# weiyithu/PV-RAFT

Hardware: NVIDIA H100
Metric: raft_sample_iters_per_sec (higher is better)
Workload: dtype f32

## Files before the change

### pvraft_b200/csrc/common.cuh

```cuda
#pragma once
#include <cstdlib>
#include <cuda_runtime.h>
#include <stdint.h>
#include <stdio.h>

#include "../../include/pvraft_b200.h"

namespace pvraft {

constexpr int kWarp = 32;
constexpr unsigned kFull = 0xffffffffu;
constexpr int kSmemBudget = 227 * 1024;

void set_error(const char* fmt, ...);
int fail(int code, const char* fmt, ...);
int check_launch(const char* what);
int sm_count();

template <typename Kernel>
inline int opt_in_smem(Kernel k, size_t bytes) {
    if (bytes > (size_t)kSmemBudget) return fail(PVRAFT_ERR_SMEM, "kernel needs %zu B of shared memory (> %d)", bytes, kSmemBudget);
    cudaError_t e = cudaFuncSetAttribute(k, cudaFuncAttributeMaxDynamicSharedMemorySize, (int)bytes);
    if (e != cudaSuccess) return fail((int)e, "cudaFuncSetAttribute(smem=%zu): %s", bytes, cudaGetErrorString(e));
    return 0;
}

__device__ __forceinline__ int lane_id() { return threadIdx.x & 31; }
__device__ __forceinline__ int warp_id() { return threadIdx.x >> 5; }

__device__ __forceinline__ float warp_max(float v) {
#pragma unroll
    for (int o = 16; o > 0; o >>= 1) v = fmaxf(v, __shfl_xor_sync(kFull, v, o));
    return v;
}
__device__ __forceinline__ float warp_min(float v) {
#pragma unroll
    for (int o = 16; o > 0; o >>= 1) v = fminf(v, __shfl_xor_sync(kFull, v, o));
    return v;
}
__device__ __forceinline__ double warp_sum(double v) {
#pragma unroll
    for (int o = 16; o > 0; o >>= 1) v += __shfl_xor_sync(kFull, v, o);
    return v;
}
__device__ __forceinline__ float warp_sum(float v) {
#pragma unroll
    for (int o = 16; o > 0; o >>= 1) v += __shfl_xor_sync(kFull, v, o);
    return v;
}

__device__ __forceinline__ float4 ld_stream_f4(const float4* p) {
    float4 r;
    asm volatile("ld.global.nc.L1::no_allocate.v4.f32 {%0,%1,%2,%3}, [%4];" : "=f"(r.x), "=f"(r.y), "=f"(r.z), "=f"(r.w) : "l"(p));
    return r;
}
__device__ __forceinline__ int4 ld_stream_i4(const int4* p) {
    int4 r;
    asm volatile("ld.global.nc.L1::no_allocate.v4.s32 {%0,%1,%2,%3}, [%4];" : "=r"(r.x), "=r"(r.y), "=r"(r.z), "=r"(r.w) : "l"(p));
    return r;
}

struct GnAffine {
    float scale, shift;
};
__device__ __forceinline__ GnAffine gn_affine(const double* stats_bg , double count,
                                              float gamma, float beta) {
    const double mean = stats_bg[0] / count;
    double var = stats_bg[1] / count - mean * mean;
    var = var < 0.0 ? 0.0 : var;
    const double rstd = rsqrt(var + 1e-5);
    GnAffine a;
    a.scale = (float)(rstd * (double)gamma);
    a.shift = (float)((double)beta - mean * rstd * (double)gamma);
    return a;
}

__device__ __forceinline__ void kahan_add(float& s, float& err, float y) {
    const float v = y - err, t = s + v;
    err = (t - s) - v;
    s = t;
}
__device__ __forceinline__ double kahan_value(float s, float err) { return (double)s - (double)err; }
__device__ __forceinline__ double pivot_sumsq(double sum_y, float p, float sdd, int n) {
    const double dp = p;
    return fma(dp, 2.0 * sum_y - (double)n * dp, (double)sdd);
}

__device__ __forceinline__ float apply_act(float x, int act, float slope) {
    if (act == PVRAFT_ACT_RELU) return fmaxf(x, 0.f);
    if (act == PVRAFT_ACT_LRELU) return x >= 0.f ? x : slope * x;
    return x;
}

struct ActCoef {
    float lo, slope;
};
__device__ __forceinline__ ActCoef act_coef(int act, float slope) {
    ActCoef c;
    c.lo = act == PVRAFT_ACT_NONE ? -INFINITY : 0.f;
    c.slope = act == PVRAFT_ACT_LRELU ? slope : 0.f;
    return c;
}
__device__ __forceinline__ float apply_act(float x, const ActCoef& c) { return fmaf(c.slope, fminf(x, 0.f), fmaxf(x, c.lo)); }

__device__ __forceinline__ float4 tc_gn_act4(float4 x, const float4& sc, const float4& sh, const ActCoef& act) {
    x.x = apply_act(fmaf(x.x, sc.x, sh.x), act);
    x.y = apply_act(fmaf(x.y, sc.y, sh.y), act);
    x.z = apply_act(fmaf(x.z, sc.z, sh.z), act);
    x.w = apply_act(fmaf(x.w, sc.w, sh.w), act);
    return x;
}

__device__ __forceinline__ float tsigmoid(float x) { return 1.f / (1.f + expf(-x)); }
__device__ __forceinline__ float tgru_blend(float z, float h, float q_pre) { return (1.f - z) * h + z * tanhf(q_pre); }

__host__ __device__ __forceinline__ void split_range(long long total, int parts, int w, long long& begin, long long& end) {
    const long long per = (total + parts - 1) / parts;
    begin = per * w;
    end = begin + per;
    if (begin > total) begin = total;
    if (end > total) end = total;
}

__device__ __forceinline__ void pdl_trigger() { asm volatile("griddepcontrol.launch_dependents;" ::: "memory"); }
__device__ __forceinline__ void pdl_wait() { asm volatile("griddepcontrol.wait;" ::: "memory"); }
template <typename... KArgs, typename... Args>
inline cudaError_t launch_pdl(void (*kernel)(KArgs...), int grid, int block, size_t smem, cudaStream_t stream, Args... args) {
    cudaLaunchConfig_t cfg{};
    cfg.gridDim = dim3((unsigned)grid);
    cfg.blockDim = dim3((unsigned)block);
    cfg.dynamicSmemBytes = smem;
    cfg.stream = stream;
    cudaLaunchAttribute attr[1];
    attr[0].id = cudaLaunchAttributeProgrammaticStreamSerialization;
    attr[0].val.programmaticStreamSerializationAllowed = 1;
    cfg.attrs = attr;
    cfg.numAttrs = 1;
    return cudaLaunchKernelEx(&cfg, kernel, KArgs(args)...);
}

}
```

### pvraft_b200/csrc/update_chain.cu

```cuda
#include "tma.cuh"
#include "wgmma.cuh"

namespace pvraft {

constexpr int kChThreads = 288;
constexpr int kChProducerWarp = 8;
constexpr int kChWBytes = 128 * kTcKB * 4;
template <bool BF16> struct ChRing {
    static constexpr int stages = BF16 ? 4 : 2;
    static constexpr int w_off = BF16 ? kTcABytes + 2 * kTcABf16Bytes : 2 * kTcABytes;
    static constexpr int stage_bytes = BF16 ? w_off + kChWBytes / 2 : w_off + 2 * kChWBytes;
};
constexpr int kChBufBytes = 2 * kTcABytes;
constexpr int kChSteps = 24;
enum ChSrc { CH_Y1 = 0, CH_KFEAT, CH_CFLOW, CH_NET, CH_INP, CH_X, CH_Y };

struct ChainParams {
    const double* y1_stats;
    const float *gn_gamma, *gn_beta;
    double gn_count;
    float gn_slope;
    const float *flow, *net;
    const float *b_cc, *b_m, *b_z, *b_r, *b_q;
    float *net_out, *p_out;
    int M, pts_per_sample;
};
struct ChainMaps {
    CUtensorMap a[5];
    CUtensorMap w_hi[5], w_lo[5];
};

__device__ __forceinline__ int ch_layer(int i) { return i < 6 ? 0 : i < 10 ? 1 : i < 16 ? 2 : i < 22 ? 3 : 4; }
__device__ __forceinline__ int ch_src(int i) {
    constexpr unsigned long long pairs = (unsigned long long)CH_X | (unsigned long long)CH_CFLOW << 4 | (unsigned long long)CH_NET << 8 |
                                         (unsigned long long)CH_INP << 12 | (unsigned long long)CH_Y << 16 | (unsigned long long)CH_X << 20 |
                                         (unsigned long long)CH_INP << 24 | (unsigned long long)CH_Y << 28 | (unsigned long long)CH_X << 32;
    return i < 4 ? CH_Y1 : i < 6 ? CH_KFEAT : (int)((pairs >> (4 * ((i - 6) >> 1))) & 15u);
}
__device__ __forceinline__ int ch_skb(int i) {
    return i < 4 ? i : (i < 6 ? i - 4 : (i - 6) & 1);
}
__device__ __forceinline__ int ch_first(int layer) { return layer == 0 ? 0 : layer == 1 ? 6 : layer == 2 ? 10 : layer == 3 ? 16 : 22; }
__device__ __forceinline__ int ch_w_bytes(int layer, bool bf16) { return (layer == 2 ? 128 : 64) * kTcKB * (bf16 ? 2 : 4); }

__device__ __forceinline__ void ch_buf_store2(unsigned char* buf, int r, int c, float v0, float v1) {
    const int lc = (c & 31) >> 2;
    *reinterpret_cast<float2*>(buf + (c >> 5) * kTcABytes + r * 128 + ((lc ^ (r & 7)) << 4) + (c & 3) * 4) = make_float2(v0, v1);
}

template <int N, bool BF16>
__device__ __forceinline__ void ch_kblock(float (&acc)[64], int kb, int src, int skb, unsigned char* tiles, unsigned char* buf_x,
                                          unsigned char* buf_y, const float* g_scale, const float* g_shift, const ActCoef& iact,
                                          unsigned long long* s_full, unsigned long long* s_empty, TcCursor& cp, int grp, int t,
                                          int lane) {
    const int s = cp.s;
    mbar_wait(&s_full[s], cp.phase);
    unsigned char* st = tiles + (size_t)s * ChRing<BF16>::stage_bytes;
    const unsigned char* from = src == CH_X ? buf_x + skb * kTcABytes : src == CH_Y ? buf_y + skb * kTcABytes : st;
#pragma unroll
    for (int i = 0; i < 4; ++i) {
        const int c = t + i * 128, r = grp * 64 + (c >> 3), lc = c & 7;
        const int off = r * 128 + ((lc ^ (r & 7)) << 4);
        float4 x = *reinterpret_cast<const float4*>(from + off);
        if (src == CH_Y1) {
            const int k = skb * kTcKB + lc * 4;
            x = tc_gn_act4(x, *reinterpret_cast<const float4*>(g_scale + k), *reinterpret_cast<const float4*>(g_shift + k), iact);
        }
        if constexpr (BF16) tc_bf16_store(st + kTcABytes + grp * kTcABf16Bytes, c >> 3, lc, x);
        else tc_split_store(st, off, x);
    }
    asm volatile("fence.proxy.async.shared::cta;" ::: "memory");
    asm volatile("bar.sync %0, 128;" ::"r"(1 + grp) : "memory");
    const unsigned char* wb = st + ChRing<BF16>::w_off;
    wgmma_fence_regs(acc);
    wgmma_fence();
    if constexpr (BF16) tc_mma_kblock_bf16<N>(acc, wgmma_desc_bf16(st + kTcABytes + grp * kTcABf16Bytes), wgmma_desc_bf16(wb), kb);
    else tc_mma_kblock<N>(acc, wgmma_desc(st + grp * 64 * 128), wgmma_desc(st + kTcABytes + grp * 64 * 128), wgmma_desc(wb),
                          wgmma_desc(wb + N * kTcKB * 4), kb);
    wgmma_commit();
    wgmma_wait<0>();
    if (lane == 0) mbar_arrive(&s_empty[s]);
    cp.next(kChSteps, ChRing<BF16>::stages);
}
template <int N, bool BF16>
__device__ __forceinline__ void ch_layer_mma(float (&acc)[64], int i0, int nkb, unsigned char* tiles, unsigned char* buf_x,
                                             unsigned char* buf_y, const float* g_scale, const float* g_shift, const ActCoef& iact,
                                             unsigned long long* s_full, unsigned long long* s_empty, TcCursor& cp, int grp, int t,
                                             int lane) {
    for (int kb = 0; kb < nkb; ++kb)
        ch_kblock<N, BF16>(acc, kb, ch_src(i0 + kb), ch_skb(i0 + kb), tiles, buf_x, buf_y, g_scale, g_shift, iact, s_full, s_empty, cp, grp, t, lane);
    wgmma_fence_regs(acc);
}

template <bool BF16>
__global__ void __launch_bounds__(kChThreads, 1)
k_update_chain(const __grid_constant__ ChainMaps maps, const ChainParams p) {
    constexpr int kChStages = ChRing<BF16>::stages, kChStageBytes = ChRing<BF16>::stage_bytes;
    extern __shared__ __align__(1024) unsigned char smem_raw[];
    unsigned char* tiles = SMEM_ALIGN_1024(smem_raw);
    unsigned char* buf_x = tiles + (size_t)kChStages * kChStageBytes;
    unsigned char* buf_y = buf_x + kChBufBytes;
    float* s_scale = reinterpret_cast<float*>(buf_y + kChBufBytes);
    float* s_bias = s_scale + 2 * 256;
    __shared__ __align__(8) unsigned long long s_full[kChStages], s_empty[kChStages];
    const int warp = warp_id(), lane = lane_id();
    const int n_tiles = p.M / kTcM;
    const int my_tiles = blockIdx.x < n_tiles ? (n_tiles - 1 - blockIdx.x) / gridDim.x + 1 : 0;
    if (warp == kChProducerWarp && lane == 0) {
        for (int i = 0; i < 5; ++i) {
            prefetch_tensormap(&maps.a[i]);
            prefetch_tensormap(&maps.w_hi[i]);
            if constexpr (!BF16) prefetch_tensormap(&maps.w_lo[i]);
        }
        for (int s = 0; s < kChStages; ++s) { mbar_init(&s_full[s], 1); mbar_init(&s_empty[s], 8); }
        fence_mbarrier_init();
    }
    asm volatile("griddepcontrol.launch_dependents;" ::: "memory");
    __syncthreads();
    asm volatile("griddepcontrol.wait;" ::: "memory");
    if (threadIdx.x < 64) {
        const int c = threadIdx.x;
        s_bias[c] = __ldg(p.b_cc + c);
        s_bias[64 + c] = c < 61 ? __ldg(p.b_m + c) : 0.f;
        s_bias[128 + c] = __ldg(p.b_z + c);
        s_bias[192 + c] = __ldg(p.b_r + c);
        s_bias[256 + c] = __ldg(p.b_q + c);
    }
    __syncthreads();

    if (warp == kChProducerWarp) {
        if (lane == 0) {
            TcCursor cw;
            for (int step = 0; step < my_tiles * kChSteps; ++step, cw.next(kChSteps, kChStages)) {
                const int i = cw.kb, layer = ch_layer(i), src = ch_src(i);
                const int row0 = (blockIdx.x + cw.ti * gridDim.x) * kTcM;
                const int wb = ch_w_bytes(layer, BF16);
                const int lkb = i - ch_first(layer), skb = ch_skb(i);
                mbar_wait(&s_empty[cw.s], cw.phase ^ 1u);
                unsigned char* st = tiles + (size_t)cw.s * kChStageBytes;
                mbar_expect_tx(&s_full[cw.s], (unsigned)((src < CH_X ? kTcABytes : 0) + (BF16 ? 1 : 2) * wb));
                if (src < CH_X) tma_load_2d(st, &maps.a[src], &s_full[cw.s], skb * kTcKB, row0);
                tma_load_2d(st + ChRing<BF16>::w_off, &maps.w_hi[layer], &s_full[cw.s], lkb * kTcKB, 0);
                if constexpr (!BF16) tma_load_2d(st + ChRing<BF16>::w_off + wb, &maps.w_lo[layer], &s_full[cw.s], lkb * kTcKB, 0);
            }
        }
        return;
    }

    const int grp = warp >> 2, t = threadIdx.x & 127;
    float* g_scale = s_scale + grp * 256;
    float* g_shift = g_scale + 128;
    const ActCoef iact = act_coef(PVRAFT_ACT_LRELU, p.gn_slope);
    const ActCoef relu = act_coef(PVRAFT_ACT_RELU, 0.f), none = act_coef(PVRAFT_ACT_NONE, 0.f);
    const int tiles_per_sample = p.pts_per_sample / kTcM;
    const int rq = (warp & 3) * 16 + (lane >> 2);
    const int cq = 2 * (lane & 3);
    int table_sample = -1;
    TcCursor cp;
    float acc[64], z[32];
    for (int ti = 0; ti < my_tiles; ++ti) {
        const int tile = blockIdx.x + ti * gridDim.x;
        const int row0 = tile * kTcM;
        const int sample = tile / tiles_per_sample;
        if (sample != table_sample) {
            table_sample = sample;
            asm volatile("bar.sync %0, 128;" ::"r"(1 + grp) : "memory");
            const double* sp = p.y1_stats + (size_t)sample * 16 + (t / 16) * 2;
            const double st[2] = {__ldcg(sp), __ldcg(sp + 1)};
            const GnAffine af = gn_affine(st, p.gn_count, __ldg(p.gn_gamma + t), __ldg(p.gn_beta + t));
            g_scale[t] = af.scale;
            g_shift[t] = af.shift;
            asm volatile("bar.sync %0, 128;" ::"r"(1 + grp) : "memory");
        }
        const int r_lo = grp * 64 + rq;
        ch_layer_mma<64, BF16>(acc, 0, 6, tiles, buf_x, buf_y, g_scale, g_shift, iact, s_full, s_empty, cp, grp, t, lane);
#pragma unroll
        for (int j = 0; j < 8; ++j)
#pragma unroll
            for (int h = 0; h < 2; ++h) {
                const int c = 8 * j + cq;
                ch_buf_store2(buf_x, r_lo + 8 * h, c, apply_act(acc[4 * j + 2 * h] + s_bias[c], relu), apply_act(acc[4 * j + 2 * h + 1] + s_bias[c + 1], relu));
            }
        asm volatile("bar.sync %0, 128;" ::"r"(1 + grp) : "memory");
        ch_layer_mma<64, BF16>(acc, 6, 4, tiles, buf_x, buf_y, g_scale, g_shift, iact, s_full, s_empty, cp, grp, t, lane);
#pragma unroll
        for (int j = 0; j < 8; ++j)
#pragma unroll
            for (int h = 0; h < 2; ++h) {
                const int c = 8 * j + cq, r = r_lo + 8 * h;
                float v0 = apply_act(acc[4 * j + 2 * h] + s_bias[64 + c], relu), v1 = apply_act(acc[4 * j + 2 * h + 1] + s_bias[64 + c + 1], relu);
                if (c >= 60) {
                    const float* fl = p.flow + (size_t)(row0 + r) * 3;
                    if (c == 62) { v0 = __ldcg(fl + 1); v1 = __ldcg(fl + 2); } else { v1 = __ldcg(fl); }
                }
                ch_buf_store2(buf_y, r, c, v0, v1);
            }
        asm volatile("bar.sync %0, 128;" ::"r"(1 + grp) : "memory");
        ch_layer_mma<128, BF16>(acc, 10, 6, tiles, buf_x, buf_y, g_scale, g_shift, iact, s_full, s_empty, cp, grp, t, lane);
#pragma unroll
        for (int j = 0; j < 8; ++j)
#pragma unroll
            for (int h = 0; h < 2; ++h) {
                const int c = 8 * j + cq, r = r_lo + 8 * h;
                const float2 hv = __ldcg(reinterpret_cast<const float2*>(p.net + (size_t)(row0 + r) * 64 + c));
                z[4 * j + 2 * h] = tsigmoid(acc[4 * j + 2 * h] + s_bias[128 + c]);
                z[4 * j + 2 * h + 1] = tsigmoid(acc[4 * j + 2 * h + 1] + s_bias[128 + c + 1]);
                ch_buf_store2(buf_x, r, c, tsigmoid(acc[32 + 4 * j + 2 * h] + s_bias[192 + c]) * hv.x,
                              tsigmoid(acc[32 + 4 * j + 2 * h + 1] + s_bias[192 + c + 1]) * hv.y);
            }
        asm volatile("bar.sync %0, 128;" ::"r"(1 + grp) : "memory");
        ch_layer_mma<64, BF16>(acc, 16, 6, tiles, buf_x, buf_y, g_scale, g_shift, iact, s_full, s_empty, cp, grp, t, lane);
#pragma unroll
        for (int j = 0; j < 8; ++j)
#pragma unroll
            for (int h = 0; h < 2; ++h) {
                const int c = 8 * j + cq, r = r_lo + 8 * h;
                const size_t g = (size_t)(row0 + r) * 64 + c;
                const float2 hv = __ldcg(reinterpret_cast<const float2*>(p.net + g));
                const float o0 = tgru_blend(z[4 * j + 2 * h], hv.x, acc[4 * j + 2 * h] + s_bias[256 + c]);
                const float o1 = tgru_blend(z[4 * j + 2 * h + 1], hv.y, acc[4 * j + 2 * h + 1] + s_bias[256 + c + 1]);
                *reinterpret_cast<float2*>(p.net_out + g) = make_float2(o0, o1);
                ch_buf_store2(buf_x, r, c, o0, o1);
            }
        asm volatile("bar.sync %0, 128;" ::"r"(1 + grp) : "memory");
        ch_layer_mma<64, BF16>(acc, 22, 2, tiles, buf_x, buf_y, g_scale, g_shift, iact, s_full, s_empty, cp, grp, t, lane);
#pragma unroll
        for (int j = 0; j < 8; ++j)
#pragma unroll
            for (int h = 0; h < 2; ++h) {
                const int c = 8 * j + cq, r = r_lo + 8 * h;
                *reinterpret_cast<float2*>(p.p_out + (size_t)(row0 + r) * 64 + c) =
                    make_float2(apply_act(acc[4 * j + 2 * h] + 0.f, none), apply_act(acc[4 * j + 2 * h + 1] + 0.f, none));
            }
    }
}

}

using namespace pvraft;

extern "C" int pvraft_update_chain_fwd(const pvraft_update_chain_args* a, void* stream) {
    if (!a || !a->y1 || !a->y1_stats || !a->gn_gamma || !a->gn_beta || !a->kfeat || !a->cflow || !a->flow || !a->net || !a->inp ||
        !a->b_cc || !a->b_m || !a->b_z || !a->b_r || !a->b_q || !a->net_out || !a->p_out)
        return fail(PVRAFT_ERR_BAD_ARG, "update_chain: null pointer");
    const bool bf16 = a->w_bf16[0] != nullptr;
    for (int l = 0; l < 5; ++l) {
        if (bf16 ? (!a->w_bf16[l] || a->w_hi[l] || a->w_lo[l]) : (!a->w_hi[l] || !a->w_lo[l] || a->w_bf16[l]))
            return fail(PVRAFT_ERR_BAD_ARG, "update_chain: layer %d needs w_hi and w_lo (3xTF32) or w_bf16 (bf16), as every other layer", l);
    }
    if (a->B <= 0 || a->N <= 0) return fail(PVRAFT_ERR_BAD_ARG, "update_chain: bad shape (B=%d, N=%d)", a->B, a->N);
    if (a->N % kTcM) return fail(PVRAFT_ERR_UNSUPPORTED, "update_chain: points per sample (%d) must be a multiple of 128", a->N);
    if (a->hidden != 64 || a->context != 64 || a->y1_channels != 128)
        return fail(PVRAFT_ERR_UNSUPPORTED, "update_chain: built for hidden = context = 64 and 128 lookup features (got %d, %d, %d)",
                    a->hidden, a->context, a->y1_channels);
    if (a->net_out == a->net) return fail(PVRAFT_ERR_BAD_ARG, "update_chain: net_out must not alias net");
    const long long M = (long long)a->B * a->N;
    ChainMaps maps;
    const float* src[5] = {a->y1, a->kfeat, a->cflow, a->net, a->inp};
    const int width[5] = {128, 64, 64, 64, 64};
    const int n_pad[5] = {64, 64, 128, 64, 64}, k[5] = {192, 128, 192, 192, 64};
    int rc;
    for (int i = 0; i < 5; ++i) {
        if ((rc = make_tensor_map(&maps.a[i], src[i], M, width[i], width[i], kTcM, "update_chain"))) return rc;
        if (bf16) {
            if ((rc = make_tensor_map_bf16(&maps.w_hi[i], a->w_bf16[i], n_pad[i], k[i], k[i], n_pad[i], "update_chain"))) return rc;
            maps.w_lo[i] = maps.w_hi[i];
        } else if ((rc = make_tensor_map(&maps.w_hi[i], a->w_hi[i], n_pad[i], k[i], k[i], n_pad[i], "update_chain")) ||
                   (rc = make_tensor_map(&maps.w_lo[i], a->w_lo[i], n_pad[i], k[i], k[i], n_pad[i], "update_chain"))) {
            return rc;
        }
    }
    ChainParams p{};
    p.y1_stats = a->y1_stats; p.gn_gamma = a->gn_gamma; p.gn_beta = a->gn_beta; p.gn_count = a->gn_count; p.gn_slope = a->gn_slope;
    p.flow = a->flow; p.net = a->net;
    p.b_cc = a->b_cc; p.b_m = a->b_m; p.b_z = a->b_z; p.b_r = a->b_r; p.b_q = a->b_q;
    p.net_out = a->net_out; p.p_out = a->p_out;
    p.M = (int)M; p.pts_per_sample = a->N;
    const size_t ring = bf16 ? (size_t)ChRing<true>::stages * ChRing<true>::stage_bytes : (size_t)ChRing<false>::stages * ChRing<false>::stage_bytes;
    const size_t smem = ring + 2 * kChBufBytes + (2 * 256 + 5 * 64) * sizeof(float) + 1024;
    const auto kernel = bf16 ? k_update_chain<true> : k_update_chain<false>;
    if ((rc = opt_in_smem(kernel, smem))) return rc;
    const long long n_tiles = M / kTcM;
    const int grid = (int)(n_tiles < sm_count() ? n_tiles : sm_count());
    const cudaError_t le = launch_pdl(kernel, grid, kChThreads, smem, (cudaStream_t)stream, maps, p);
    if (le != cudaSuccess) return fail((int)le, "update_chain: launch failed: %s", cudaGetErrorString(le));
    return check_launch("update_chain");
}
```

Baseline: 9922.

## Keep one wgmma in flight per k-block, prefetch flow/net, add fast sigmoid path

In the BF16 path, each k-block now waits only until one wgmma group remains in flight and releases the previous ring stage rather than the current one, so the next MMA can overlap with the wait. The last k-block of each layer still drains fully. Flow and net values are loaded into registers ahead of the epilogues instead of inside the store loops. The gate sigmoid uses an approximate reciprocal with one Newton step when all inputs for the thread are above -80, falling back to the exact version otherwise. This trades higher register pressure and more complex stage-release bookkeeping for less stall time.

After: 9897, median of 6. No clear change (-0.3%).

```diff
diff --git a/pvraft_b200/csrc/common.cuh b/pvraft_b200/csrc/common.cuh
--- a/pvraft_b200/csrc/common.cuh
+++ b/pvraft_b200/csrc/common.cuh
@@ -112,6 +112,13 @@
 }
 
 __device__ __forceinline__ float tsigmoid(float x) { return 1.f / (1.f + expf(-x)); }
+constexpr float kSigmoidFastMin = -80.f;
+__device__ __forceinline__ float tsigmoid_fast(float x) {
+    const float d = 1.f + expf(-x);
+    float r;
+    asm("rcp.approx.ftz.f32 %0, %1;" : "=f"(r) : "f"(d));
+    return fmaf(r, -fmaf(d, r, -1.f), r);
+}
 __device__ __forceinline__ float tgru_blend(float z, float h, float q_pre) { return (1.f - z) * h + z * tanhf(q_pre); }
 
 __host__ __device__ __forceinline__ void split_range(long long total, int parts, int w, long long& begin, long long& end) {
diff --git a/pvraft_b200/csrc/update_chain.cu b/pvraft_b200/csrc/update_chain.cu
--- a/pvraft_b200/csrc/update_chain.cu
+++ b/pvraft_b200/csrc/update_chain.cu
@@ -48,7 +48,7 @@
     *reinterpret_cast<float2*>(buf + (c >> 5) * kTcABytes + r * 128 + ((lc ^ (r & 7)) << 4) + (c & 3) * 4) = make_float2(v0, v1);
 }
 
-template <int N, bool BF16>
+template <int N, bool BF16, bool LAST>
 __device__ __forceinline__ void ch_kblock(float (&acc)[64], int kb, int src, int skb, unsigned char* tiles, unsigned char* buf_x,
                                           unsigned char* buf_y, const float* g_scale, const float* g_shift, const ActCoef& iact,
                                           unsigned long long* s_full, unsigned long long* s_empty, TcCursor& cp, int grp, int t,
@@ -78,17 +78,35 @@
     else tc_mma_kblock<N>(acc, wgmma_desc(st + grp * 64 * 128), wgmma_desc(st + kTcABytes + grp * 64 * 128), wgmma_desc(wb),
                           wgmma_desc(wb + N * kTcKB * 4), kb);
     wgmma_commit();
-    wgmma_wait<0>();
-    if (lane == 0) mbar_arrive(&s_empty[s]);
+    const int prev = s == 0 ? ChRing<BF16>::stages - 1 : s - 1;
+    if (BF16 && !LAST) {
+        wgmma_wait<1>();
+        if (lane == 0 && kb > 0) mbar_arrive(&s_empty[prev]);
+    } else {
+        wgmma_wait<0>();
+        if (lane == 0) {
+            if (BF16 && kb > 0) mbar_arrive(&s_empty[prev]);
+            mbar_arrive(&s_empty[s]);
+        }
+    }
     cp.next(kChSteps, ChRing<BF16>::stages);
+}
+__device__ __forceinline__ void ch_load_net(float2 (&hv)[16], const float* net, int row0, int r_lo, int cq) {
+#pragma unroll
+    for (int j = 0; j < 8; ++j)
+#pragma unroll
+        for (int h = 0; h < 2; ++h) hv[2 * j + h] = __ldcg(reinterpret_cast<const float2*>(net + (size_t)(row0 + r_lo + 8 * h) * 64 + 8 * j + cq));
 }
 template <int N, bool BF16>
 __device__ __forceinline__ void ch_layer_mma(float (&acc)[64], int i0, int nkb, unsigned char* tiles, unsigned char* buf_x,
                                              unsigned char* buf_y, const float* g_scale, const float* g_shift, const ActCoef& iact,
                                              unsigned long long* s_full, unsigned long long* s_empty, TcCursor& cp, int grp, int t,
                                              int lane) {
-    for (int kb = 0; kb < nkb; ++kb)
-        ch_kblock<N, BF16>(acc, kb, ch_src(i0 + kb), ch_skb(i0 + kb), tiles, buf_x, buf_y, g_scale, g_shift, iact, s_full, s_empty, cp, grp, t, lane);
+    for (int kb = 0; kb < nkb - 1; ++kb)
+        ch_kblock<N, BF16, false>(acc, kb, ch_src(i0 + kb), ch_skb(i0 + kb), tiles, buf_x, buf_y, g_scale, g_shift, iact, s_full, s_empty,
+                                  cp, grp, t, lane);
+    ch_kblock<N, BF16, true>(acc, nkb - 1, ch_src(i0 + nkb - 1), ch_skb(i0 + nkb - 1), tiles, buf_x, buf_y, g_scale, g_shift, iact, s_full,
+                             s_empty, cp, grp, t, lane);
     wgmma_fence_regs(acc);
 }
 
@@ -182,6 +200,11 @@
                 ch_buf_store2(buf_x, r_lo + 8 * h, c, apply_act(acc[4 * j + 2 * h] + s_bias[c], relu), apply_act(acc[4 * j + 2 * h + 1] + s_bias[c + 1], relu));
             }
         asm volatile("bar.sync %0, 128;" ::"r"(1 + grp) : "memory");
+        float fl[2][3];
+#pragma unroll
+        for (int h = 0; h < 2; ++h)
+#pragma unroll
+            for (int k = 0; k < 3; ++k) fl[h][k] = __ldcg(p.flow + (size_t)(row0 + r_lo + 8 * h) * 3 + k);
         ch_layer_mma<64, BF16>(acc, 6, 4, tiles, buf_x, buf_y, g_scale, g_shift, iact, s_full, s_empty, cp, grp, t, lane);
 #pragma unroll
         for (int j = 0; j < 8; ++j)
@@ -190,35 +213,47 @@
                 const int c = 8 * j + cq, r = r_lo + 8 * h;
                 float v0 = apply_act(acc[4 * j + 2 * h] + s_bias[64 + c], relu), v1 = apply_act(acc[4 * j + 2 * h + 1] + s_bias[64 + c + 1], relu);
                 if (c >= 60) {
-                    const float* fl = p.flow + (size_t)(row0 + r) * 3;
-                    if (c == 62) { v0 = __ldcg(fl + 1); v1 = __ldcg(fl + 2); } else { v1 = __ldcg(fl); }
+                    if (c == 62) { v0 = fl[h][1]; v1 = fl[h][2]; } else { v1 = fl[h][0]; }
                 }
                 ch_buf_store2(buf_y, r, c, v0, v1);
             }
         asm volatile("bar.sync %0, 128;" ::"r"(1 + grp) : "memory");
         ch_layer_mma<128, BF16>(acc, 10, 6, tiles, buf_x, buf_y, g_scale, g_shift, iact, s_full, s_empty, cp, grp, t, lane);
-#pragma unroll
-        for (int j = 0; j < 8; ++j)
-#pragma unroll
-            for (int h = 0; h < 2; ++h) {
-                const int c = 8 * j + cq, r = r_lo + 8 * h;
-                const float2 hv = __ldcg(reinterpret_cast<const float2*>(p.net + (size_t)(row0 + r) * 64 + c));
-                z[4 * j + 2 * h] = tsigmoid(acc[4 * j + 2 * h] + s_bias[128 + c]);
-                z[4 * j + 2 * h + 1] = tsigmoid(acc[4 * j + 2 * h + 1] + s_bias[128 + c + 1]);
-                ch_buf_store2(buf_x, r, c, tsigmoid(acc[32 + 4 * j + 2 * h] + s_bias[192 + c]) * hv.x,
-                              tsigmoid(acc[32 + 4 * j + 2 * h + 1] + s_bias[192 + c + 1]) * hv.y);
-            }
+        float2 hv[16];
+        ch_load_net(hv, p.net, row0, r_lo, cq);
+        bool fast = true;
+#pragma unroll
+        for (int j = 0; j < 8; ++j)
+#pragma unroll
+            for (int k = 0; k < 4; ++k) {
+                const int c = 8 * j + cq + (k & 1);
+                fast &= (acc[4 * j + k] + s_bias[128 + c] >= kSigmoidFastMin) & (acc[32 + 4 * j + k] + s_bias[192 + c] >= kSigmoidFastMin);
+            }
+        const auto gates = [&](auto sigmoid) {
+#pragma unroll
+            for (int j = 0; j < 8; ++j)
+#pragma unroll
+                for (int h = 0; h < 2; ++h) {
+                    const int c = 8 * j + cq, i = 4 * j + 2 * h;
+                    z[i] = sigmoid(acc[i] + s_bias[128 + c]);
+                    z[i + 1] = sigmoid(acc[i + 1] + s_bias[128 + c + 1]);
+                    ch_buf_store2(buf_x, r_lo + 8 * h, c, sigmoid(acc[32 + i] + s_bias[192 + c]) * hv[2 * j + h].x,
+                                  sigmoid(acc[32 + i + 1] + s_bias[192 + c + 1]) * hv[2 * j + h].y);
+                }
+        };
+        if (fast) gates([](float x) { return tsigmoid_fast(x); });
+        else gates([](float x) { return tsigmoid(x); });
         asm volatile("bar.sync %0, 128;" ::"r"(1 + grp) : "memory");
         ch_layer_mma<64, BF16>(acc, 16, 6, tiles, buf_x, buf_y, g_scale, g_shift, iact, s_full, s_empty, cp, grp, t, lane);
+        ch_load_net(hv, p.net, row0, r_lo, cq);
 #pragma unroll
         for (int j = 0; j < 8; ++j)
 #pragma unroll
             for (int h = 0; h < 2; ++h) {
                 const int c = 8 * j + cq, r = r_lo + 8 * h;
                 const size_t g = (size_t)(row0 + r) * 64 + c;
-                const float2 hv = __ldcg(reinterpret_cast<const float2*>(p.net + g));
-                const float o0 = tgru_blend(z[4 * j + 2 * h], hv.x, acc[4 * j + 2 * h] + s_bias[256 + c]);
-                const float o1 = tgru_blend(z[4 * j + 2 * h + 1], hv.y, acc[4 * j + 2 * h + 1] + s_bias[256 + c + 1]);
+                const float o0 = tgru_blend(z[4 * j + 2 * h], hv[2 * j + h].x, acc[4 * j + 2 * h] + s_bias[256 + c]);
+                const float o1 = tgru_blend(z[4 * j + 2 * h + 1], hv[2 * j + h].y, acc[4 * j + 2 * h + 1] + s_bias[256 + c + 1]);
                 *reinterpret_cast<float2*>(p.net_out + g) = make_float2(o0, o1);
                 ch_buf_store2(buf_x, r, c, o0, o1);
             }
```
